# yurimjeon1892/EFGH

Hardware: AMD Instinct MI355X
Metric: frame-pairs/sec EFGHNet fwd+bwd (384x1280 RGB + 64x2048 range), whole job (higher is better)
Workload: dtype f32; 1 GPU; BASELINE.json configs[2]: EFGHNet fwd+bwd with efghloss + gradient all-reduce + fused Adam, synthetic 384x1280 RGB + 131072-point sweep, batch=8 per GPU, random-init weights; global_batch=8, points=131072, parallelism=dp1

## Files before the change

efgh_amd/csrc/gemm.hip:

```cpp
#include "common.h"
#include <type_traits>

namespace {

typedef float f32x16 __attribute__((ext_vector_type(16)));
constexpr int BK = 32;
constexpr int LDS_LD = BK + 4;
struct KArgs {
    const float *A; int64_t lda;
    int C, T, K;
    unsigned magicC;
    int Hin, Win, Hv, Wv, sh, sw;
    unsigned long long dhpack, dwpack;
    int Ho, Wo, osh, osw, oh0, ow0;
    const int *table;
    const float *W; int N;
    int tld;
    long long M; const int *M_dev;
    const float *bias, *scale, *shift, *residual; int64_t ldr;
    int act; float slope;
    float *out; int64_t ldo;
    float *stats;
    unsigned nbx;
    unsigned nbatch;
    long long bsA, bsW, bsO;
    int bsT;
    int tam;
};

template <int MODE, int BM, int BN, int WM, int WN>
__device__ __forceinline__ void gemm_epilogue(const KArgs &p, const long long M, const long long m0, const int n0, const unsigned tile_m,
                                              f32x16 (&acc)[BM / WM / 32][BN / WN / 32], const long long *rowout, float *scratch,
                                              const int wm, const int wn, const int l31, const int lh, const int tid) {
    constexpr int MI = BM / WM / 32, NI = BN / WN / 32;
    float *As = scratch;
    float *ssum = As;
    float *ssq = As + WM * BN;
    float bi[NI], sc[NI], sf[NI], s1[NI], s2[NI];
    bool cok[NI];
#pragma unroll
    for (int j = 0; j < NI; ++j) {
        const int col = n0 + (wn * NI + j) * 32 + l31;
        cok[j] = col < p.N;
        bi[j] = (p.bias && cok[j]) ? p.bias[col] : 0.f;
        sc[j] = (p.scale && cok[j]) ? p.scale[col] : 1.f;
        sf[j] = (p.shift && cok[j]) ? p.shift[col] : 0.f;
        s1[j] = 0.f; s2[j] = 0.f;
    }
    const int colb = n0 + wn * NI * 32 + l31;
    const float neg = p.act == 1 ? 0.f : (p.act == 2 ? p.slope : 1.f);
    auto rows = [&](auto res_c, auto full_c) {
        constexpr bool RES = decltype(res_c)::value, FULL = decltype(full_c)::value;
#pragma unroll
        for (int i = 0; i < MI; ++i) {
#pragma unroll
            for (int r = 0; r < 16; ++r) {
                const int rl = (wm * MI + i) * 32 + (r & 3) + 8 * (r >> 2) + 4 * lh;
                const long long orow = rowout[rl];
                if (!FULL && orow < 0) continue;
                float *op = p.out + orow * p.ldo + colb;
                float rv[NI];
                if (RES) {
                    const float *rp = p.residual + orow * p.ldr + colb;
#pragma unroll
                    for (int j = 0; j < NI; ++j) rv[j] = (FULL || cok[j]) ? rp[j * 32] : 0.f;
                }
#pragma unroll
                for (int j = 0; j < NI; ++j) {
                    float v = acc[i][j][r] + bi[j];
                    if (FULL || cok[j]) { s1[j] += v; s2[j] = fmaf(v, v, s2[j]); }
                    v = v * sc[j] + sf[j];
                    if (RES) v += rv[j];
                    v = act_neg(v, neg);
                    if (FULL || cok[j]) st_out(op + j * 32, v);
                }
            }
        }
    };
    const bool fulln = n0 + BN <= p.N && m0 + BM <= M;
    if (fulln && !p.bias && !p.scale && !p.shift && !p.residual && !p.stats && p.act == 0) {
#pragma unroll
        for (int i = 0; i < MI; ++i) {
#pragma unroll
            for (int r = 0; r < 16; ++r) {
                const int rl = (wm * MI + i) * 32 + (r & 3) + 8 * (r >> 2) + 4 * lh;
                float *op = p.out + rowout[rl] * p.ldo + colb;
#pragma unroll
                for (int j = 0; j < NI; ++j) st_out(op + j * 32, acc[i][j][r]);
            }
        }
    } else if (p.residual) {
        if (fulln) rows(std::true_type{}, std::true_type{});
        else rows(std::true_type{}, std::false_type{});
    } else {
        if (fulln) rows(std::false_type{}, std::true_type{});
        else rows(std::false_type{}, std::false_type{});
    }
    if (p.stats) {
#pragma unroll
        for (int j = 0; j < NI; ++j) {
            const int coll = (wn * NI + j) * 32 + l31;
            s1[j] += __shfl_xor(s1[j], 32); s2[j] += __shfl_xor(s2[j], 32);
            if (lh == 0) { ssum[wm * BN + coll] = s1[j]; ssq[wm * BN + coll] = s2[j]; }
        }
    }
    if (p.stats) {
        __syncthreads();
        for (int c = tid; c < BN; c += 256) {
            if (n0 + c < p.N) {
                float a = 0.f, b = 0.f;
#pragma unroll
                for (int w = 0; w < WM; ++w) { a += ssum[w * BN + c]; b += ssq[w * BN + c]; }
                p.stats[((long long)tile_m * 2 + 0) * p.N + n0 + c] = a;
                p.stats[((long long)tile_m * 2 + 1) * p.N + n0 + c] = b;
            }
        }
    }
}

template <int MODE, int BM, int BN, int WM, int WN>
__global__ void __launch_bounds__(256, 3)
k_gather_gemm(const KArgs p_in) {
    constexpr int MI = BM / WM / 32, NI = BN / WN / 32;
    constexpr int NA = BM / 32, NB = BN / 32;
    __shared__ __attribute__((aligned(16))) float As[BM * LDS_LD];
    __shared__ __attribute__((aligned(16))) float Bs[BN * LDS_LD];
    __shared__ long long rowout[BM];

    KArgs p = p_in;
    if (blockIdx.y) {
        p.A += blockIdx.y * p.bsA; p.W += blockIdx.y * p.bsW; p.out += blockIdx.y * p.bsO;
        if (MODE == 2) p.table += blockIdx.y * p.bsT;
    }
    const int tid = threadIdx.x, lane = tid & 63, wave = tid >> 6;
    const int wm = wave / WN, wn = wave % WN;
    const int l31 = lane & 31, lh = lane >> 5;
    long long M = p.M;
    if (p.M_dev) { long long md = *p.M_dev; M = md < M ? md : M; }
    const unsigned nbx = p.nbx, nblk = gridDim.x;
    const unsigned q8 = nblk >> 3, r8 = nblk & 7, xcd = blockIdx.x & 7, within = blockIdx.x >> 3;
    const unsigned lin = (xcd < r8 ? xcd * (q8 + 1) : r8 * (q8 + 1) + (xcd - r8) * q8) + within;
    const unsigned tile_m = lin / nbx, tile_n = lin - tile_m * nbx;
    const long long m0 = (long long)tile_m * BM;
    const int n0 = tile_n * BN;
    if (m0 >= M) return;

    const int arow = tid >> 3, kv = (tid & 7) * 4;
    long long abase[NA];
    unsigned amask[NA];
#pragma unroll
    for (int q = 0; q < NA; ++q) {
        long long m = m0 + q * 32 + arow;
        const bool ok = m < M;
        abase[q] = 0;
        amask[q] = 0;
        if (ok) {
            if (MODE == 0) { abase[q] = m * p.lda; amask[q] = 1; }
            else if (MODE == 4) { abase[q] = m * p.tld; amask[q] = 1; }
            else if (MODE == 2) {
                abase[q] = m * 16;
                amask[q] = 0xFFFFu;
                if (p.tam) amask[q] = (0x7FFFu & ~(unsigned)p_in.table[m * 16 + 15]) >> (blockIdx.y * p.bsT);
            }
            else if (MODE == 3) {
                long long b = m / p.Wv; int j = (int)(m - b * p.Wv);
                abase[q] = b * p.Hin * p.Win + j; amask[q] = 1;
            } else {
                int j = (int)(m % p.Wv); long long r = m / p.Wv;
                int i = (int)(r % p.Hv); long long b = r / p.Hv;
                const int ih0 = i * p.sh, iw0 = j * p.sw;
                abase[q] = ((b * p.Hin + ih0) * p.Win + iw0) * p.lda;
                unsigned mk = 0;
                for (int t = 0; t < p.T; ++t) {
                    int ih = ih0 + (int)((p.dhpack >> (4 * t)) & 15) - 8, iw = iw0 + (int)((p.dwpack >> (4 * t)) & 15) - 8;
                    if ((unsigned)ih < (unsigned)p.Hin && (unsigned)iw < (unsigned)p.Win) mk |= 1u << t;
                }
                amask[q] = mk;
            }
        }
    }
    for (int r = tid; r < BM; r += 256) {
        long long m = m0 + r, o = -1;
        if (m < M) {
            if (MODE == 1) {
                int j = (int)(m % p.Wv); long long rr = m / p.Wv;
                int i = (int)(rr % p.Hv); long long b = rr / p.Hv;
                o = (b * p.Ho + (i * p.osh + p.oh0)) * p.Wo + (j * p.osw + p.ow0);
            } else o = m;
        }
        rowout[r] = o;
    }
    long long bbase[NB]; bool bval[NB];
#pragma unroll
    for (int q = 0; q < NB; ++q) {
        int n = n0 + q * 32 + arow;
        bval[q] = n < p.N;
        bbase[q] = (long long)n * p.K;
    }

    float4 ra[NA], rb[NB];
    auto load_chunk = [&](int k0) {
        const int kk = k0 + kv;
        const bool kin = kk < p.K;
        int t = (int)(((unsigned long long)kk * p.magicC) >> 32);
        int c = kk - t * p.C;
        if (MODE == 1) {
            const int dh = (int)((p.dhpack >> (4 * (t & 15))) & 15) - 8, dw = (int)((p.dwpack >> (4 * (t & 15))) & 15) - 8;
            const long long dl = ((long long)dh * p.Win + dw) * p.lda + c;
#pragma unroll
            for (int q = 0; q < NA; ++q) {
                const bool ok = kin && ((amask[q] >> t) & 1u);
                const long long off = ok ? abase[q] + dl : 0;
                float4 v = *reinterpret_cast<const float4 *>(p.A + off);
                ra[q] = ok ? v : make_float4(0.f, 0.f, 0.f, 0.f);
            }
        } else if (MODE == 3) {
            const long long delta = (long long)t * p.Win;
#pragma unroll
            for (int q = 0; q < NA; ++q) {
                const bool ok = kin && amask[q];
                float4 v = *reinterpret_cast<const float4 *>(p.A + (ok ? (abase[q] + delta) * p.lda + c : 0));
                ra[q] = ok ? v : make_float4(0.f, 0.f, 0.f, 0.f);
            }
        } else {
#pragma unroll
            for (int q = 0; q < NA; ++q) {
                float4 v = make_float4(0.f, 0.f, 0.f, 0.f);
                if (kin && (MODE == 2 ? ((amask[q] >> t) & 1u) : amask[q])) {
                    if (MODE == 0) {
                        v = *reinterpret_cast<const float4 *>(p.A + abase[q] + kk);
                    } else {
                        int r = p.table[abase[q] + t];
                        if (r >= 0) v = *reinterpret_cast<const float4 *>(p.A + (long long)r * p.lda + c);
                    }
                }
                ra[q] = v;
            }
        }
#pragma unroll
        for (int q = 0; q < NB; ++q) {
            const bool ok = bval[q] && kin;
            float4 v = *reinterpret_cast<const float4 *>(p.W + (ok ? bbase[q] + kk : 0));
            rb[q] = ok ? v : make_float4(0.f, 0.f, 0.f, 0.f);
        }
    };

    f32x16 acc[MI][NI];
#pragma unroll
    for (int i = 0; i < MI; ++i)
#pragma unroll
        for (int j = 0; j < NI; ++j)
#pragma unroll
            for (int r = 0; r < 16; ++r) acc[i][j][r] = 0.f;

    const int nchunks = (p.K + BK - 1) / BK;
    load_chunk(0);
    for (int ch = 0; ch < nchunks; ++ch) {
#pragma unroll
        for (int q = 0; q < NA; ++q)
            *reinterpret_cast<float4 *>(&As[(q * 32 + arow) * LDS_LD + kv]) = ra[q];
#pragma unroll
        for (int q = 0; q < NB; ++q)
            *reinterpret_cast<float4 *>(&Bs[(q * 32 + arow) * LDS_LD + kv]) = rb[q];
        __syncthreads();
        if (ch + 1 < nchunks) load_chunk((ch + 1) * BK);
        const int kleft = p.K - ch * BK;
#pragma unroll
        for (int g = 0; g < 4; ++g) {
            if (g * 8 >= kleft) continue;
            float4 a[MI], b[NI];
#pragma unroll
            for (int i = 0; i < MI; ++i)
                a[i] = *reinterpret_cast<const float4 *>(
                    &As[((wm * MI + i) * 32 + l31) * LDS_LD + g * 8 + lh * 4]);
#pragma unroll
            for (int j = 0; j < NI; ++j)
                b[j] = *reinterpret_cast<const float4 *>(
                    &Bs[((wn * NI + j) * 32 + l31) * LDS_LD + g * 8 + lh * 4]);
#pragma unroll
            for (int i = 0; i < MI; ++i)
#pragma unroll
                for (int j = 0; j < NI; ++j) {
                    acc[i][j] = __builtin_amdgcn_mfma_f32_32x32x2f32(a[i].x, b[j].x, acc[i][j], 0, 0, 0);
                    acc[i][j] = __builtin_amdgcn_mfma_f32_32x32x2f32(a[i].y, b[j].y, acc[i][j], 0, 0, 0);
                    acc[i][j] = __builtin_amdgcn_mfma_f32_32x32x2f32(a[i].z, b[j].z, acc[i][j], 0, 0, 0);
                    acc[i][j] = __builtin_amdgcn_mfma_f32_32x32x2f32(a[i].w, b[j].w, acc[i][j], 0, 0, 0);
                }
        }
        __syncthreads();
    }

    gemm_epilogue<MODE, BM, BN, WM, WN>(p, M, m0, n0, tile_m, acc, rowout, As, wm, wn, l31, lh, tid);
}

__device__ __attribute__((aligned(128))) float g_gemm_zero[32];

constexpr int DMA_BM = 128;

template <int MODE, int BN>
__global__ void __launch_bounds__(256, 2)
k_gather_gemm_dma(const KArgs p_in) {
    constexpr int BM = DMA_BM, WM = 2, WN = 2, MI = 2, NI = BN / WN / 32, NBP = BN / 32;
    constexpr int STAGE = (BM + BN) * BK;
    extern __shared__ __attribute__((aligned(1024))) float ring[];
    __shared__ long long rowout[BM];

    KArgs p = p_in;
    if (blockIdx.y) { p.A += blockIdx.y * p.bsA; p.W += blockIdx.y * p.bsW; p.out += blockIdx.y * p.bsO; }
    const int tid = threadIdx.x, lane = tid & 63, wave = __builtin_amdgcn_readfirstlane(tid >> 6);
    const int wm = wave / WN, wn = wave % WN, l31 = lane & 31, lh = lane >> 5;
    const unsigned ring_lds = lds_addr(ring);
    const long long M = p.M;
    const unsigned nbx = p.nbx, nblk = gridDim.x;
    const unsigned q8 = nblk >> 3, r8 = nblk & 7, xcd = blockIdx.x & 7, within = blockIdx.x >> 3;
    const unsigned lin = (xcd < r8 ? xcd * (q8 + 1) : r8 * (q8 + 1) + (xcd - r8) * q8) + within;
    const unsigned tile_m = lin / nbx, tile_n = lin - tile_m * nbx;
    const long long m0 = (long long)tile_m * BM;
    const int n0 = tile_n * BN;
    if (m0 >= M) return;

    long long abase[4]; unsigned amask[4];
    const float *srcW[NBP];
    const int sub = lane >> 3;
#pragma unroll
    for (int q = 0; q < 4; ++q) {
        const int r = (wave * 4 + q) * 8 + sub;
        const int kq = (lane & 7) ^ ((r >> 1) & 7);
        const long long m = m0 + r;
        abase[q] = kq * 4; amask[q] = 0;
        if (m < M) {
            if (MODE == 0) { abase[q] += m * p.lda; amask[q] = 1; }
            else {
                const int j = (int)(m % p.Wv); const long long rr = m / p.Wv;
                const int i = (int)(rr % p.Hv); const long long b = rr / p.Hv;
                const int ih0 = i * p.sh, iw0 = j * p.sw;
                abase[q] += ((b * p.Hin + ih0) * p.Win + iw0) * p.lda;
                unsigned mk = 0;
                for (int t = 0; t < p.T; ++t) {
                    const int ih = ih0 + (int)((p.dhpack >> (4 * t)) & 15) - 8, iw = iw0 + (int)((p.dwpack >> (4 * t)) & 15) - 8;
                    if ((unsigned)ih < (unsigned)p.Hin && (unsigned)iw < (unsigned)p.Win) mk |= 1u << t;
                }
                amask[q] = mk;
            }
        }
    }
#pragma unroll
    for (int q = 0; q < NBP; ++q) {
        const int r = (wave * NBP + q) * 8 + sub;
        const int kq = (lane & 7) ^ ((r >> 1) & 7);
        int n = n0 + r;
        if (n >= p.N) n = p.N - 1;
        srcW[q] = p.W + (long long)n * p.K + kq * 4;
    }
    for (int r = tid; r < BM; r += 256) {
        const long long m = m0 + r;
        long long o = -1;
        if (m < M) {
            if (MODE == 1) {
                const int j = (int)(m % p.Wv); const long long rr = m / p.Wv;
                const int i = (int)(rr % p.Hv); const long long b = rr / p.Hv;
                o = (b * p.Ho + (i * p.osh + p.oh0)) * p.Wo + (j * p.osw + p.ow0);
            } else o = m;
        }
        rowout[r] = o;
    }
    const float *zsrc = g_gemm_zero + (lane & 7) * 4;
    auto issue = [&](int chunk, int buf) {
        const unsigned base = ring_lds + (unsigned)(buf * STAGE) * 4u;
        const int k0 = chunk * BK;
        const int t = (int)(((unsigned long long)k0 * p.magicC) >> 32);
        const int c = k0 - t * p.C;
        long long dl = c;
        if (MODE == 1) {
            const int dh = (int)((p.dhpack >> (4 * (t & 15))) & 15) - 8, dw = (int)((p.dwpack >> (4 * (t & 15))) & 15) - 8;
            dl += ((long long)dh * p.Win + dw) * p.lda;
        }
#pragma unroll
        for (int q = 0; q < 4; ++q) {
            const bool ok = MODE == 0 ? amask[q] != 0 : ((amask[q] >> t) & 1u) != 0;
            dma16(ok ? p.A + abase[q] + dl : zsrc, base + (unsigned)((wave * 4 + q) * 1024));
        }
#pragma unroll
        for (int q = 0; q < NBP; ++q) dma16(srcW[q] + k0, base + (unsigned)(BM * BK * 4 + (wave * NBP + q) * 1024));
    };

    int offA[MI], offW[NI], swA[MI], swW[NI];
#pragma unroll
    for (int i = 0; i < MI; ++i) { const int ra = (wm * MI + i) * 32 + l31; offA[i] = ra * BK; swA[i] = (ra >> 1) & 7; }
#pragma unroll
    for (int j = 0; j < NI; ++j) { const int rw = (wn * NI + j) * 32 + l31; offW[j] = BM * BK + rw * BK; swW[j] = (rw >> 1) & 7; }

    f32x16 acc[MI][NI];
#pragma unroll
    for (int i = 0; i < MI; ++i)
#pragma unroll
        for (int j = 0; j < NI; ++j)
#pragma unroll
            for (int r = 0; r < 16; ++r) acc[i][j][r] = 0.f;

    const int nch = p.K / BK;
    issue(0, 0);
    for (int ch = 0; ch < nch; ++ch) {
        wait_vm<0>();
        __builtin_amdgcn_s_barrier();
        asm volatile("" ::: "memory");
        if (ch + 1 < nch) issue(ch + 1, (ch + 1) & 1);
        const float *buf = ring + (ch & 1) * STAGE;
        float4 a[2][MI], b[2][NI];
        auto frag = [&](int g, float4 (&fa)[MI], float4 (&fb)[NI]) {
#pragma unroll
            for (int i = 0; i < MI; ++i) fa[i] = *reinterpret_cast<const float4 *>(buf + offA[i] + (((g * 2 + lh) ^ swA[i]) << 2));
#pragma unroll
            for (int j = 0; j < NI; ++j) fb[j] = *reinterpret_cast<const float4 *>(buf + offW[j] + (((g * 2 + lh) ^ swW[j]) << 2));
        };
        frag(0, a[0], b[0]);
#pragma unroll
        for (int g = 0; g < 4; ++g) {
            if (g < 3) frag(g + 1, a[(g + 1) & 1], b[(g + 1) & 1]);
            __builtin_amdgcn_sched_barrier(0);
            const float4 (&ca)[MI] = a[g & 1];
            const float4 (&cb)[NI] = b[g & 1];
#pragma unroll
            for (int i = 0; i < MI; ++i)
#pragma unroll
                for (int j = 0; j < NI; ++j) {
                    acc[i][j] = __builtin_amdgcn_mfma_f32_32x32x2f32(ca[i].x, cb[j].x, acc[i][j], 0, 0, 0);
                    acc[i][j] = __builtin_amdgcn_mfma_f32_32x32x2f32(ca[i].y, cb[j].y, acc[i][j], 0, 0, 0);
                    acc[i][j] = __builtin_amdgcn_mfma_f32_32x32x2f32(ca[i].z, cb[j].z, acc[i][j], 0, 0, 0);
                    acc[i][j] = __builtin_amdgcn_mfma_f32_32x32x2f32(ca[i].w, cb[j].w, acc[i][j], 0, 0, 0);
                }
            __builtin_amdgcn_sched_barrier(0);
        }
    }
    __syncthreads();
    gemm_epilogue<MODE, BM, BN, WM, WN>(p, M, m0, n0, tile_m, acc, rowout, ring, wm, wn, l31, lh, tid);
}

__global__ void k_pack_weight(const float *__restrict__ W, float *__restrict__ Wp, int N, int T, int C, int Nw, int Cw,
                              long long sn, long long sc, long long st, const int4 taps0,
                              const int4 taps1, const int4 taps2, const int4 taps3) {
    const int tp[16] = {taps0.x, taps0.y, taps0.z, taps0.w, taps1.x, taps1.y, taps1.z, taps1.w,
                        taps2.x, taps2.y, taps2.z, taps2.w, taps3.x, taps3.y, taps3.z, taps3.w};
    long long total = (long long)N * T * C;
    for (long long i = (long long)blockIdx.x * blockDim.x + threadIdx.x; i < total;
         i += (long long)gridDim.x * blockDim.x) {
        int c = (int)(i % C); long long r = i / C;
        int t = (int)(r % T); int n = (int)(r / T);
        int ti = 0;
#pragma unroll
        for (int q = 0; q < 16; ++q) if (q == t) ti = tp[q];
        Wp[i] = (n < Nw && c < Cw) ? W[n * sn + c * sc + ti * st] : 0.f;
    }
}

__global__ void __launch_bounds__(256) k_pack_weight_batched(const efgh_pack_job *__restrict__ jobs, const long long *__restrict__ prefix,
                                                             int njobs, long long total) {
    __shared__ int job_s;
    for (long long i0 = (long long)blockIdx.x * 256; i0 < total; i0 += (long long)gridDim.x * 256) {
        if (threadIdx.x == 0) {
            int lo = 0, hi = njobs - 1;
            while (lo < hi) { const int mid = (lo + hi + 1) >> 1; if (prefix[mid] <= i0) lo = mid; else hi = mid - 1; }
            job_s = lo;
        }
        __syncthreads();
        int jb = job_s;
        __syncthreads();
        const long long i = i0 + threadIdx.x;
        if (i >= total) continue;
        while (jb + 1 < njobs && prefix[jb + 1] <= i) ++jb;
        const efgh_pack_job &j = jobs[jb];
        const long long e = i - prefix[jb];
        int n, t, c;
        if (e < 0x7fffffffLL) {
            const unsigned eu = (unsigned)e, r = eu / (unsigned)j.Cp;
            c = (int)(eu - r * (unsigned)j.Cp); n = (int)(r / (unsigned)j.T); t = (int)(r - (unsigned)n * (unsigned)j.T);
        } else {
            c = (int)(e % j.Cp); const long long r = e / j.Cp;
            t = (int)(r % j.T); n = (int)(r / j.T);
        }
        j.Wp[e] = (n < j.N && c < j.C) ? j.W[n * j.sn + c * j.sc + j.taps[t] * j.st] : 0.f;
    }
}

constexpr int PK_TN = 8, PK_TC = 32;
__global__ void __launch_bounds__(256) k_pack_weight_tiled(const efgh_pack_job *__restrict__ jobs, const long long *__restrict__ tile_prefix,
                                                           int njobs) {
    __shared__ float tile[PK_TN * 16 * (PK_TC + 1)];
    __shared__ int job_s;
    if (threadIdx.x == 0) {
        int lo = 0, hi = njobs - 1;
        while (lo < hi) { const int mid = (lo + hi + 1) >> 1; if (tile_prefix[mid] <= (long long)blockIdx.x) lo = mid; else hi = mid - 1; }
        job_s = lo;
    }
    __syncthreads();
    const efgh_pack_job &j = jobs[job_s];
    const int T = j.T, Np = j.Np, Cp = j.Cp;
    const int ctiles = (Cp + PK_TC - 1) / PK_TC;
    const int tl = (int)((long long)blockIdx.x - tile_prefix[job_s]);
    const int n0 = (tl / ctiles) * PK_TN, c0 = (tl % ctiles) * PK_TC;
    const int nelem = PK_TN * PK_TC * T;
    const bool c_inner = j.sc <= j.sn;
    for (int e = threadIdx.x; e < nelem; e += 256) {
        const int t = e % T, r = e / T;
        int n, c;
        if (c_inner) { c = r % PK_TC; n = r / PK_TC; }
        else { n = r % PK_TN; c = r / PK_TN; }
        const int gn = n0 + n, gc = c0 + c;
        float v = 0.f;
        if (gn < j.N && gc < j.C) v = j.W[gn * j.sn + gc * j.sc + j.taps[t] * j.st];
        tile[(n * T + t) * (PK_TC + 1) + c] = v;
    }
    __syncthreads();
    for (int e = threadIdx.x; e < nelem; e += 256) {
        const int c = e % PK_TC, r = e / PK_TC;
        const int n = r / T, t = r - n * T;
        const int gn = n0 + n, gc = c0 + c;
        if (gn < Np && gc < Cp) j.Wp[((long long)gn * T + t) * Cp + gc] = tile[r * (PK_TC + 1) + c];
    }
}

__global__ void k_fold_planes(const float4 *__restrict__ part, int S, long long M, int N4, const float4 *__restrict__ bias, int act,
                              float slope, float *__restrict__ out, long long ldo) {
    const long long total = M * N4;
    for (long long i = (long long)blockIdx.x * blockDim.x + threadIdx.x; i < total; i += (long long)gridDim.x * blockDim.x) {
        const long long m = i / N4; const int n4 = (int)(i - m * N4);
        float4 a = part[i];
        for (int z = 1; z < S; ++z) { const float4 b = part[(long long)z * total + i]; a.x += b.x; a.y += b.y; a.z += b.z; a.w += b.w; }
        if (bias) { const float4 b = bias[n4]; a.x += b.x; a.y += b.y; a.z += b.z; a.w += b.w; }
        if (act == 1) { a.x = fmaxf(a.x, 0.f); a.y = fmaxf(a.y, 0.f); a.z = fmaxf(a.z, 0.f); a.w = fmaxf(a.w, 0.f); }
        else if (act == 2) {
            a.x = a.x > 0.f ? a.x : a.x * slope; a.y = a.y > 0.f ? a.y : a.y * slope;
            a.z = a.z > 0.f ? a.z : a.z * slope; a.w = a.w > 0.f ? a.w : a.w * slope;
        }
        *reinterpret_cast<float4 *>(out + m * ldo + n4 * 4) = a;
    }
}

__global__ void k_pad_vec(const float *__restrict__ v, int n, float *__restrict__ out, int np, float fill) {
    const int i = blockIdx.x * blockDim.x + threadIdx.x;
    if (i < np) out[i] = i < n ? v[i] : fill;
}

template <int MODE, int BM, int BN, int WM, int WN>
void launch(const KArgs &a0, hipStream_t st) {
    KArgs a = a0;
    a.nbx = (unsigned)((a.N + BN - 1) / BN);
    const long long nby = (a.M + BM - 1) / BM;
    k_gather_gemm<MODE, BM, BN, WM, WN><<<dim3((unsigned)(a.nbx * nby), a.nbatch), 256, 0, st>>>(a);
}

std::atomic<unsigned long long> g_dma_raised[4];
bool g_use_dma = true;

bool dma_ok(const KArgs &a, int mode) {
    return g_use_dma && (mode == 0 || mode == 1) && a.N > 32 && a.C % 32 == 0 && !a.M_dev && a.lda % 4 == 0 && a.K % BK == 0
           && (((uintptr_t)a.A) & 15) == 0 && (((uintptr_t)a.W) & 15) == 0;
}

template <int MODE, int BN>
int launch_dma(const KArgs &a0, hipStream_t st) {
    KArgs a = a0;
    a.nbx = (unsigned)((a.N + BN - 1) / BN);
    const long long nby = (a.M + DMA_BM - 1) / DMA_BM;
    const size_t lds = (size_t)2 * (DMA_BM + BN) * BK * sizeof(float);
    if (!efgh_raise_lds_once(g_dma_raised[MODE * 2 + (BN == 128)], (const void *)k_gather_gemm_dma<MODE, BN>, (int)lds)) {
        efgh_set_error("%s:%d: cannot raise the dynamic LDS limit of k_gather_gemm_dma", __FILE__, __LINE__);
        return EFGH_E_LAUNCH;
    }
    k_gather_gemm_dma<MODE, BN><<<dim3((unsigned)(a.nbx * nby), a.nbatch), 256, lds, st>>>(a);
    return EFGH_OK;
}

template <int MODE>
int dispatch(const KArgs &a, hipStream_t st) {
    if constexpr (MODE == 0 || MODE == 1) {
        if (dma_ok(a, MODE)) return a.N > 64 ? launch_dma<MODE, 128>(a, st) : launch_dma<MODE, 64>(a, st);
    }
    if (a.N > 64) launch<MODE, 128, 128, 2, 2>(a, st);
    else if (a.N > 32) launch<MODE, 128, 64, 2, 2>(a, st);
    else launch<MODE, 256, 32, 4, 1>(a, st);
    return EFGH_OK;
}

int tile_m(int N) { return N > 32 ? 128 : 256; }

}

extern "C" int32_t efgh_gather_gemm_grid_m(int64_t M, int32_t N) {
    int bm = tile_m(N);
    return (int32_t)((M + bm - 1) / bm);
}

static int fill_args(const efgh_gemm_desc *d, KArgs &a, int tld = 0) {
    EFGH_CHECK_ARG(d && d->A && d->W && d->out);
    EFGH_CHECK_ARG(d->C > 0 && d->C % 4 == 0 && d->T >= 1 && (d->T <= 16 || d->mode == 3 || tld > 0));
    EFGH_CHECK_ARG(d->N >= 1 && d->M >= 1 && d->lda % 4 == 0);
    EFGH_CHECK_ARG((((uintptr_t)d->A) & 15) == 0 && (((uintptr_t)d->W) & 15) == 0);
    EFGH_CHECK_ARG(d->mode >= 0 && d->mode <= 3);
    EFGH_CHECK_ARG((int64_t)d->T * d->C < 65536);
    a.A = d->A; a.lda = d->lda; a.C = d->C; a.T = d->T; a.K = d->T * d->C;
    a.magicC = (unsigned)((0x100000000ULL + d->C - 1) / d->C);
    a.Hin = d->Hin; a.Win = d->Win; a.Hv = d->Hv; a.Wv = d->Wv; a.sh = d->sh; a.sw = d->sw;
    a.dhpack = 0; a.dwpack = 0;
    for (int t = 0; t < 16; ++t) {
        int dh = t < d->T ? d->dh[t] : 0, dw = t < d->T ? d->dw[t] : 0;
        if (d->mode == 1) EFGH_CHECK_ARG(dh >= -8 && dh <= 7 && dw >= -8 && dw <= 7);
        a.dhpack |= (unsigned long long)((dh + 8) & 15) << (4 * t);
        a.dwpack |= (unsigned long long)((dw + 8) & 15) << (4 * t);
    }
    a.Ho = d->Ho; a.Wo = d->Wo; a.osh = d->osh; a.osw = d->osw; a.oh0 = d->oh0; a.ow0 = d->ow0;
    a.table = d->table; a.W = d->W; a.N = d->N; a.M = d->M; a.M_dev = d->M_dev;
    a.bias = d->bias; a.scale = d->scale; a.shift = d->shift; a.residual = d->residual; a.ldr = d->ldr;
    a.act = d->act; a.slope = d->slope; a.out = d->out; a.ldo = d->ldo; a.stats = d->stats;
    a.nbatch = d->nbatch > 1 ? (unsigned)d->nbatch : 1u;
    a.bsA = d->batch_stride_a; a.bsW = d->batch_stride_w; a.bsO = d->batch_stride_out; a.bsT = d->batch_stride_table;
    a.tam = d->mode == 2 ? d->table_alias_mask : 0;
    if (a.nbatch > 1) EFGH_CHECK_ARG(!d->stats && !d->residual && a.nbatch <= 65535 && a.bsA % 4 == 0 && a.bsW % 4 == 0);
    if (d->mode == 1) {
        EFGH_CHECK_ARG(d->B > 0 && d->Hin > 0 && d->Win > 0 && d->Hv > 0 && d->Wv > 0);
        EFGH_CHECK_ARG(d->M == (int64_t)d->B * d->Hv * d->Wv);
        EFGH_CHECK_ARG(d->osh >= 1 && d->osw >= 1 && d->Ho > 0 && d->Wo > 0);
    }
    a.tld = tld;
    if (tld > 0) EFGH_CHECK_ARG(d->mode == 2 && d->table != nullptr && tld >= d->T && a.nbatch == 1 && !d->table_alias_mask);
    else if (d->mode == 2) EFGH_CHECK_ARG(d->table != nullptr && d->batch_stride_table >= 0 && (int64_t)d->batch_stride_table * (a.nbatch - 1) + d->T <= 16);
    if (d->mode == 0) EFGH_CHECK_ARG(d->T == 1);
    if (d->mode == 3) EFGH_CHECK_ARG(d->B > 0 && d->Hin == d->T && d->Win > 0 && d->Wv > 0 && d->M == (int64_t)d->B * d->Wv);
    return EFGH_OK;
}

extern "C" int efgh_gather_gemm(const efgh_gemm_desc *d, void *stream_) {
    hipStream_t st = (hipStream_t)stream_;
    KArgs a;
    int rc = fill_args(d, a);
    if (rc != EFGH_OK) return rc;
    if (d->mode == 0) rc = dispatch<0>(a, st);
    else if (d->mode == 1) rc = dispatch<1>(a, st);
    else if (d->mode == 2) rc = dispatch<2>(a, st);
    else rc = dispatch<3>(a, st);
    if (rc != EFGH_OK) return rc;
    EFGH_CHECK_LAUNCH();
    return EFGH_OK;
}

extern "C" int efgh_blur_r_gemm(const efgh_gemm_desc *d, int32_t ld, void *stream_) {
    KArgs a;
    EFGH_CHECK_ARG(d && ld > 0);
    int rc = fill_args(d, a, ld);
    if (rc != EFGH_OK) return rc;
    rc = dispatch<4>(a, (hipStream_t)stream_);
    if (rc != EFGH_OK) return rc;
    EFGH_CHECK_LAUNCH();
    return EFGH_OK;
}

extern "C" int efgh_gather_gemm_set_dma(int32_t on) {
    const int old = g_use_dma ? 1 : 0;
    g_use_dma = on != 0;
    return old;
}

extern "C" int efgh_pack_weight_batched(const efgh_pack_job *jobs_dev, const int64_t *prefix_dev, int32_t njobs, int64_t total,
                                        void *stream_) {
    EFGH_CHECK_ARG(jobs_dev && prefix_dev && njobs > 0 && total > 0);
    long long g = (total + 255) / 256;
    k_pack_weight_batched<<<(int)(g > 16384 ? 16384 : g), 256, 0, (hipStream_t)stream_>>>(jobs_dev, (const long long *)prefix_dev, njobs,
                                                                                         total);
    EFGH_CHECK_LAUNCH();
    return EFGH_OK;
}

extern "C" int efgh_pack_weight_batched_tiled(const efgh_pack_job *jobs_dev, const int64_t *tile_prefix_dev, int32_t njobs, int64_t ntiles,
                                              void *stream_) {
    EFGH_CHECK_ARG(jobs_dev && tile_prefix_dev && njobs > 0 && ntiles > 0 && ntiles < 0x7fffffffLL);
    k_pack_weight_tiled<<<(unsigned)ntiles, 256, 0, (hipStream_t)stream_>>>(jobs_dev, (const long long *)tile_prefix_dev, njobs);
    EFGH_CHECK_LAUNCH();
    return EFGH_OK;
}

extern "C" int efgh_fold_planes(const float *part, int32_t S, int64_t M, int32_t N, const float *bias, int32_t act, float slope,
                                float *out, int64_t ldo, void *stream_) {
    EFGH_CHECK_ARG(part && out && S >= 1 && M > 0 && N > 0 && N % 4 == 0 && ldo % 4 == 0 && ldo >= N);
    EFGH_CHECK_ARG((((uintptr_t)part) & 15) == 0 && (((uintptr_t)out) & 15) == 0 && (!bias || (((uintptr_t)bias) & 15) == 0));
    const long long total = M * (N / 4);
    long long g = (total + 255) / 256;
    k_fold_planes<<<(int)(g > 8192 ? 8192 : g), 256, 0, (hipStream_t)stream_>>>((const float4 *)part, S, M, N / 4, (const float4 *)bias,
                                                                              act, slope, out, ldo);
    EFGH_CHECK_LAUNCH();
    return EFGH_OK;
}

extern "C" int efgh_pad_vec(const float *v, int32_t n, float *out, int32_t np, float fill, void *stream_) {
    EFGH_CHECK_ARG(v && out && n > 0 && np >= n);
    k_pad_vec<<<cdiv(np, 256), 256, 0, (hipStream_t)stream_>>>(v, n, out, np, fill);
    EFGH_CHECK_LAUNCH();
    return EFGH_OK;
}

extern "C" int efgh_pack_weight(const float *W, float *Wp, int32_t N, int32_t T, int32_t C, int64_t sn,
                                int64_t sc, int64_t stt, const int32_t *tapidx, void *stream_) {
    return efgh_pack_weight_padded(W, Wp, N, T, C, N, C, sn, sc, stt, tapidx, stream_);
}

extern "C" int efgh_pack_weight_padded(const float *W, float *Wp, int32_t N, int32_t T, int32_t C, int32_t Np, int32_t Cp,
                                       int64_t sn, int64_t sc, int64_t stt, const int32_t *tapidx, void *stream_) {
    hipStream_t st = (hipStream_t)stream_;
    EFGH_CHECK_ARG(W && Wp && N > 0 && T > 0 && T <= 16 && C > 0 && Np >= N && Cp >= C);
    int tp[16];
    for (int t = 0; t < 16; ++t) tp[t] = (tapidx && t < T) ? tapidx[t] : (t < T ? t : 0);
    long long total = (long long)Np * T * Cp;
    int grid = (int)((total + 255) / 256);
    if (grid > 8192) grid = 8192;
    k_pack_weight<<<grid, 256, 0, st>>>(W, Wp, Np, T, Cp, N, C, sn, sc, stt, make_int4(tp[0], tp[1], tp[2], tp[3]),
                                        make_int4(tp[4], tp[5], tp[6], tp[7]),
                                        make_int4(tp[8], tp[9], tp[10], tp[11]),
                                        make_int4(tp[12], tp[13], tp[14], tp[15]));
    EFGH_CHECK_LAUNCH();
    return EFGH_OK;
}
```

Measured before the change: 31.38 frame-pairs/s.

## Use three-stage K16 DMA ring with higher occupancy for BN=128 gather GEMM

For the wide-N DMA gather GEMM, the K step per stage is halved to 16 and the LDS ring becomes triple-buffered. The loop now waits only for the oldest stage's loads, so two chunks stay in flight. Per-block LDS shrinks, which lets the launch bound request three blocks per CU to hide memory latency. In exchange there are more barriers per K, shorter MFMA bursts between syncs, and possible register pressure from the higher occupancy target.

```diff
diff --git a/efgh_amd/csrc/gemm.hip b/efgh_amd/csrc/gemm.hip
--- a/efgh_amd/csrc/gemm.hip
+++ b/efgh_amd/csrc/gemm.hip
@@ -297,11 +297,17 @@
 
 constexpr int DMA_BM = 128;
 
+constexpr int dma_step(int BN) { return BN == 128 ? 16 : 32; }
+constexpr int dma_slots(int BN) { return BN == 128 ? 3 : 2; }
+constexpr size_t dma_lds(int BN) { return (size_t)dma_slots(BN) * (DMA_BM + BN) * dma_step(BN) * sizeof(float); }
+
 template <int MODE, int BN>
-__global__ void __launch_bounds__(256, 2)
+__global__ void __launch_bounds__(256, BN == 128 ? 3 : 2)
 k_gather_gemm_dma(const KArgs p_in) {
-    constexpr int BM = DMA_BM, WM = 2, WN = 2, MI = 2, NI = BN / WN / 32, NBP = BN / 32;
-    constexpr int STAGE = (BM + BN) * BK;
+    constexpr int BM = DMA_BM, WM = 2, WN = 2, MI = 2, NI = BN / WN / 32, KD = dma_step(BN), NBUF = dma_slots(BN);
+    constexpr int NAP = BM * KD / 1024, NBP = BN * KD / 1024;
+    constexpr int QR = KD / 4, RP = 256 / KD, SWS = KD == 32 ? 1 : 2;
+    constexpr int STAGE = (BM + BN) * KD;
     extern __shared__ __attribute__((aligned(1024))) float ring[];
     __shared__ long long rowout[BM];
 
@@ -319,13 +325,13 @@
     const int n0 = tile_n * BN;
     if (m0 >= M) return;
 
-    long long abase[4]; unsigned amask[4];
+    long long abase[NAP]; unsigned amask[NAP];
     const float *srcW[NBP];
-    const int sub = lane >> 3;
-#pragma unroll
-    for (int q = 0; q < 4; ++q) {
-        const int r = (wave * 4 + q) * 8 + sub;
-        const int kq = (lane & 7) ^ ((r >> 1) & 7);
+    const int sub = lane / QR;
+#pragma unroll
+    for (int q = 0; q < NAP; ++q) {
+        const int r = (wave * NAP + q) * RP + sub;
+        const int kq = (lane & (QR - 1)) ^ ((r >> SWS) & (QR - 1));
         const long long m = m0 + r;
         abase[q] = kq * 4; amask[q] = 0;
         if (m < M) {
@@ -346,8 +352,8 @@
     }
 #pragma unroll
     for (int q = 0; q < NBP; ++q) {
-        const int r = (wave * NBP + q) * 8 + sub;
-        const int kq = (lane & 7) ^ ((r >> 1) & 7);
+        const int r = (wave * NBP + q) * RP + sub;
+        const int kq = (lane & (QR - 1)) ^ ((r >> SWS) & (QR - 1));
         int n = n0 + r;
         if (n >= p.N) n = p.N - 1;
         srcW[q] = p.W + (long long)n * p.K + kq * 4;
@@ -364,10 +370,10 @@
         }
         rowout[r] = o;
     }
-    const float *zsrc = g_gemm_zero + (lane & 7) * 4;
+    const float *zsrc = g_gemm_zero + (lane & (QR - 1)) * 4;
     auto issue = [&](int chunk, int buf) {
         const unsigned base = ring_lds + (unsigned)(buf * STAGE) * 4u;
-        const int k0 = chunk * BK;
+        const int k0 = chunk * KD;
         const int t = (int)(((unsigned long long)k0 * p.magicC) >> 32);
         const int c = k0 - t * p.C;
         long long dl = c;
@@ -376,19 +382,19 @@
             dl += ((long long)dh * p.Win + dw) * p.lda;
         }
 #pragma unroll
-        for (int q = 0; q < 4; ++q) {
+        for (int q = 0; q < NAP; ++q) {
             const bool ok = MODE == 0 ? amask[q] != 0 : ((amask[q] >> t) & 1u) != 0;
-            dma16(ok ? p.A + abase[q] + dl : zsrc, base + (unsigned)((wave * 4 + q) * 1024));
-        }
-#pragma unroll
-        for (int q = 0; q < NBP; ++q) dma16(srcW[q] + k0, base + (unsigned)(BM * BK * 4 + (wave * NBP + q) * 1024));
+            dma16(ok ? p.A + abase[q] + dl : zsrc, base + (unsigned)((wave * NAP + q) * 1024));
+        }
+#pragma unroll
+        for (int q = 0; q < NBP; ++q) dma16(srcW[q] + k0, base + (unsigned)(BM * KD * 4 + (wave * NBP + q) * 1024));
     };
 
     int offA[MI], offW[NI], swA[MI], swW[NI];
 #pragma unroll
-    for (int i = 0; i < MI; ++i) { const int ra = (wm * MI + i) * 32 + l31; offA[i] = ra * BK; swA[i] = (ra >> 1) & 7; }
-#pragma unroll
-    for (int j = 0; j < NI; ++j) { const int rw = (wn * NI + j) * 32 + l31; offW[j] = BM * BK + rw * BK; swW[j] = (rw >> 1) & 7; }
+    for (int i = 0; i < MI; ++i) { const int ra = (wm * MI + i) * 32 + l31; offA[i] = ra * KD; swA[i] = (ra >> SWS) & (QR - 1); }
+#pragma unroll
+    for (int j = 0; j < NI; ++j) { const int rw = (wn * NI + j) * 32 + l31; offW[j] = BM * KD + rw * KD; swW[j] = (rw >> SWS) & (QR - 1); }
 
     f32x16 acc[MI][NI];
 #pragma unroll
@@ -398,14 +404,17 @@
 #pragma unroll
             for (int r = 0; r < 16; ++r) acc[i][j][r] = 0.f;
 
-    const int nch = p.K / BK;
-    issue(0, 0);
+    const int nch = p.K / KD;
+#pragma unroll
+    for (int s = 0; s < NBUF - 1; ++s)
+        if (s < nch) issue(s, s);
     for (int ch = 0; ch < nch; ++ch) {
-        wait_vm<0>();
+        if (NBUF == 2 || ch + 1 >= nch) wait_vm<0>();
+        else wait_vm<NAP + NBP>();
         __builtin_amdgcn_s_barrier();
         asm volatile("" ::: "memory");
-        if (ch + 1 < nch) issue(ch + 1, (ch + 1) & 1);
-        const float *buf = ring + (ch & 1) * STAGE;
+        if (ch + NBUF - 1 < nch) issue(ch + NBUF - 1, (ch + NBUF - 1) % NBUF);
+        const float *buf = ring + (ch % NBUF) * STAGE;
         float4 a[2][MI], b[2][NI];
         auto frag = [&](int g, float4 (&fa)[MI], float4 (&fb)[NI]) {
 #pragma unroll
@@ -415,8 +424,8 @@
         };
         frag(0, a[0], b[0]);
 #pragma unroll
-        for (int g = 0; g < 4; ++g) {
-            if (g < 3) frag(g + 1, a[(g + 1) & 1], b[(g + 1) & 1]);
+        for (int g = 0; g < KD / 8; ++g) {
+            if (g + 1 < KD / 8) frag(g + 1, a[(g + 1) & 1], b[(g + 1) & 1]);
             __builtin_amdgcn_sched_barrier(0);
             const float4 (&ca)[MI] = a[g & 1];
             const float4 (&cb)[NI] = b[g & 1];
@@ -549,7 +558,6 @@
     k_gather_gemm<MODE, BM, BN, WM, WN><<<dim3((unsigned)(a.nbx * nby), a.nbatch), 256, 0, st>>>(a);
 }
 
-std::atomic<unsigned long long> g_dma_raised[4];
 bool g_use_dma = true;
 
 bool dma_ok(const KArgs &a, int mode) {
@@ -559,11 +567,12 @@
 
 template <int MODE, int BN>
 int launch_dma(const KArgs &a0, hipStream_t st) {
+    static std::atomic<unsigned long long> raised;
     KArgs a = a0;
     a.nbx = (unsigned)((a.N + BN - 1) / BN);
     const long long nby = (a.M + DMA_BM - 1) / DMA_BM;
-    const size_t lds = (size_t)2 * (DMA_BM + BN) * BK * sizeof(float);
-    if (!efgh_raise_lds_once(g_dma_raised[MODE * 2 + (BN == 128)], (const void *)k_gather_gemm_dma<MODE, BN>, (int)lds)) {
+    constexpr size_t lds = dma_lds(BN);
+    if (!efgh_raise_lds_once(raised, (const void *)k_gather_gemm_dma<MODE, BN>, (int)lds)) {
         efgh_set_error("%s:%d: cannot raise the dynamic LDS limit of k_gather_gemm_dma", __FILE__, __LINE__);
         return EFGH_E_LAUNCH;
     }
```

New measurement: 31.31 frame-pairs/s. About the same (-0.2%).
